# Nightmare-n/GD-MAE

Hardware: AMD Instinct MI355X
Metric: MAE pre-train frames/sec (Waymo-shape, 180k pts, 75% mask) (higher is better)
Workload: dtype bf16

## Files before the change

gd-mae_amd/csrc/dw_grouped.h:

```cpp
#pragma once
#include <hip/hip_runtime.h>

#define GD_DW_MAX_JOBS 9

struct GdDwJob {
  const void* G;
  const void* X;
  int M, N;
  float* part;
  float* colpart;
  int tile0;
  const int* xidx;
  int xidx_stride;
  int x_f32;
  int g_ld, g_cols;
};
struct GdDwGroup {
  GdDwJob job[GD_DW_MAX_JOBS];
  int n_jobs;
  int tiles_total;
  int S;
  long long rows_per_slice;
  long long n_valid;
  int guard_rows = 0;
  int pair_mode = 0;
};

bool gd_dw_group_supported(long long n_pad, int d, int ff);
int gd_dw_group_slices(long long n_pad, int tiles_total);
int gd_dw_group_slices_for(long long n_pad, int tiles_total, int max_wgs);
int gd_dw_pick(long long n, int tiles_total, int max_wgs, long long* n_pad);
int gd_dw_grouped(hipStream_t st, GdDwGroup& A, long long n_pad, long long n_valid);
int gd_dw_grouped_s(hipStream_t st, GdDwGroup& A, long long n_pad, long long n_valid, int S);
```

gd-mae_amd/csrc/dw_grouped.hip:

```cpp
#include "common.h"
#include "dw_grouped.h"
#include <stdlib.h>

typedef float f32x16 __attribute__((ext_vector_type(16)));
typedef __bf16 bf16x8 __attribute__((ext_vector_type(8)));
typedef short s16x4 __attribute__((ext_vector_type(4)));

namespace {
constexpr int kTile = 128;
constexpr int kChunk = 64;
constexpr int kRowBytes = kTile * 2;
constexpr int kStage = kChunk * kRowBytes;

__device__ __forceinline__ int stage_off(int row, int u16) { return row * kRowBytes + (((u16 >> 2) ^ (row & 3)) << 6) + ((u16 & 3) << 4); }

struct Chunk {
  uint4 q0, q1, q2, q3;
};
__device__ __forceinline__ Chunk load_chunk(const unsigned short* __restrict__ p, int ld, unsigned r, unsigned last) {
  Chunk k;
  k.q0 = *reinterpret_cast<const uint4*>(p + (unsigned long long)(r < last ? r : last) * (unsigned)ld);
  k.q1 = *reinterpret_cast<const uint4*>(p + (unsigned long long)(r + 16 < last ? r + 16 : last) * (unsigned)ld);
  k.q2 = *reinterpret_cast<const uint4*>(p + (unsigned long long)(r + 32 < last ? r + 32 : last) * (unsigned)ld);
  k.q3 = *reinterpret_cast<const uint4*>(p + (unsigned long long)(r + 48 < last ? r + 48 : last) * (unsigned)ld);
  return k;
}
__device__ __forceinline__ void zero_chunk_unless(Chunk& k, unsigned keep_mask) {
  k.q0.x &= keep_mask; k.q0.y &= keep_mask; k.q0.z &= keep_mask; k.q0.w &= keep_mask;
  k.q1.x &= keep_mask; k.q1.y &= keep_mask; k.q1.z &= keep_mask; k.q1.w &= keep_mask;
  k.q2.x &= keep_mask; k.q2.y &= keep_mask; k.q2.z &= keep_mask; k.q2.w &= keep_mask;
  k.q3.x &= keep_mask; k.q3.y &= keep_mask; k.q3.z &= keep_mask; k.q3.w &= keep_mask;
}
__device__ __forceinline__ uint4 cvt_f32x8(const float4& a, const float4& b) {
  uint4 q;
  q.x = gd_pack_bf16(a.x, a.y); q.y = gd_pack_bf16(a.z, a.w);
  q.z = gd_pack_bf16(b.x, b.y); q.w = gd_pack_bf16(b.z, b.w);
  return q;
}
struct ChunkIdx {
  int j0, j1, j2, j3;
};
__device__ __forceinline__ ChunkIdx load_chunk_idx(const int* __restrict__ xidx, int stride, unsigned row0, unsigned n_valid, int tid) {
  const unsigned r = row0 + (tid >> 4), lastv = n_valid - 1;
  auto at = [&](unsigned rr) { return xidx[(unsigned long long)(rr < lastv ? rr : lastv) * (unsigned)stride]; };
  ChunkIdx k;
  k.j0 = at(r); k.j1 = at(r + 16); k.j2 = at(r + 32); k.j3 = at(r + 48);
  return k;
}
template <bool F32>
__device__ __forceinline__ Chunk load_chunk_rows(const void* __restrict__ base, int ld, const ChunkIdx& I, int col0, int tid) {
  const int col = col0 + (tid & 15) * 8;
  const long long o0 = (long long)(I.j0 < 0 ? 0 : I.j0) * ld + col, o1 = (long long)(I.j1 < 0 ? 0 : I.j1) * ld + col;
  const long long o2 = (long long)(I.j2 < 0 ? 0 : I.j2) * ld + col, o3 = (long long)(I.j3 < 0 ? 0 : I.j3) * ld + col;
  Chunk k;
  if (F32) {
    const float* f = (const float*)base;
    const float4 a0 = *reinterpret_cast<const float4*>(f + o0), b0 = *reinterpret_cast<const float4*>(f + o0 + 4);
    const float4 a1 = *reinterpret_cast<const float4*>(f + o1), b1 = *reinterpret_cast<const float4*>(f + o1 + 4);
    const float4 a2 = *reinterpret_cast<const float4*>(f + o2), b2 = *reinterpret_cast<const float4*>(f + o2 + 4);
    const float4 a3 = *reinterpret_cast<const float4*>(f + o3), b3 = *reinterpret_cast<const float4*>(f + o3 + 4);
    k.q0 = cvt_f32x8(a0, b0); k.q1 = cvt_f32x8(a1, b1); k.q2 = cvt_f32x8(a2, b2); k.q3 = cvt_f32x8(a3, b3);
  } else {
    const unsigned short* h = (const unsigned short*)base;
    k.q0 = *reinterpret_cast<const uint4*>(h + o0);
    k.q1 = *reinterpret_cast<const uint4*>(h + o1);
    k.q2 = *reinterpret_cast<const uint4*>(h + o2);
    k.q3 = *reinterpret_cast<const uint4*>(h + o3);
  }
  return k;
}
__device__ __forceinline__ unsigned missing_bits(const ChunkIdx& I) {
  return (I.j0 < 0 ? 1u : 0u) | (I.j1 < 0 ? 2u : 0u) | (I.j2 < 0 ? 4u : 0u) | (I.j3 < 0 ? 8u : 0u);
}
__device__ __forceinline__ void zero_missing(Chunk& k, unsigned bits) {
  const unsigned m0 = (bits & 1u) ? 0u : ~0u, m1 = (bits & 2u) ? 0u : ~0u, m2 = (bits & 4u) ? 0u : ~0u, m3 = (bits & 8u) ? 0u : ~0u;
  k.q0.x &= m0; k.q0.y &= m0; k.q0.z &= m0; k.q0.w &= m0;
  k.q1.x &= m1; k.q1.y &= m1; k.q1.z &= m1; k.q1.w &= m1;
  k.q2.x &= m2; k.q2.y &= m2; k.q2.z &= m2; k.q2.w &= m2;
  k.q3.x &= m3; k.q3.y &= m3; k.q3.z &= m3; k.q3.w &= m3;
}
__device__ __forceinline__ void mask_chunk(Chunk& k, long long row0, int tid, long long n_valid) {
  if (row0 + kChunk <= n_valid) return;
  const int r = tid >> 4;
  const uint4 z = make_uint4(0u, 0u, 0u, 0u);
  if (row0 + r >= n_valid) k.q0 = z;
  if (row0 + r + 16 >= n_valid) k.q1 = z;
  if (row0 + r + 32 >= n_valid) k.q2 = z;
  if (row0 + r + 48 >= n_valid) k.q3 = z;
}
__device__ __forceinline__ void store_chunk(unsigned char* __restrict__ lds, int tid, const Chunk& k) {
  const int c = tid & 15, r = tid >> 4;
  unsigned char* p = lds + stage_off(r, c);
  *reinterpret_cast<uint4*>(p) = k.q0;
  *reinterpret_cast<uint4*>(p + 16 * kRowBytes) = k.q1;
  *reinterpret_cast<uint4*>(p + 32 * kRowBytes) = k.q2;
  *reinterpret_cast<uint4*>(p + 48 * kRowBytes) = k.q3;
}
__device__ __forceinline__ void add_bf16x8(const uint4& q, float (&cs)[8]) {
  cs[0] += __uint_as_float(q.x << 16); cs[1] += __uint_as_float(q.x & 0xFFFF0000u);
  cs[2] += __uint_as_float(q.y << 16); cs[3] += __uint_as_float(q.y & 0xFFFF0000u);
  cs[4] += __uint_as_float(q.z << 16); cs[5] += __uint_as_float(q.z & 0xFFFF0000u);
  cs[6] += __uint_as_float(q.w << 16); cs[7] += __uint_as_float(q.w & 0xFFFF0000u);
}
__device__ __forceinline__ bf16x8 frag(const unsigned char* __restrict__ lds, int k0, int col32, int lane) {
  const int i = lane & 15, grp = (lane >> 4) & 1, h = lane >> 5;
  const int row = k0 + 8 * h + (i >> 2);
  const int seg = col32 >> 5;
  const unsigned char* p0 = lds + row * kRowBytes + ((seg ^ (row & 3)) << 6) + 32 * grp + 8 * (i & 3);
  const int row1 = row + 4;
  const unsigned char* p1 = lds + row1 * kRowBytes + ((seg ^ (row1 & 3)) << 6) + 32 * grp + 8 * (i & 3);
  const s16x4 lo = __builtin_amdgcn_ds_read_tr16_b64_v4i16((s16x4 __attribute__((address_space(3)))*)p0);
  const s16x4 hi = __builtin_amdgcn_ds_read_tr16_b64_v4i16((s16x4 __attribute__((address_space(3)))*)p1);
  const uint2 a = __builtin_bit_cast(uint2, lo), b = __builtin_bit_cast(uint2, hi);
  return __builtin_bit_cast(bf16x8, make_uint4(a.x, a.y, b.x, b.y));
}

template <int XM>
__global__ __launch_bounds__(256, 2) void k_dw_grouped(GdDwGroup A) {
  extern __shared__ __attribute__((aligned(16))) unsigned char lds[];
  const int tid = threadIdx.x, lane = tid & 63, wv = tid >> 6;
  const int xcd = blockIdx.x & 7, pos = blockIdx.x >> 3;
  const int sg = pos / A.tiles_total, t = pos - sg * A.tiles_total;
  const int s = sg * 8 + xcd;
  const unsigned short* G = (const unsigned short*)A.job[0].G;
  const unsigned short* X = (const unsigned short*)A.job[0].X;
  float* part = A.job[0].part;
  float* colpart = A.job[0].colpart;
  int M = A.job[0].M, N = A.job[0].N, tile0 = 0;
  const int* xidx = A.job[0].xidx;
  int xstride = A.job[0].xidx_stride, x_f32 = A.job[0].x_f32;
  int g_ld = A.job[0].g_ld, g_cols = A.job[0].g_cols;
#pragma unroll
  for (int j = 1; j < GD_DW_MAX_JOBS; ++j)
    if (j < A.n_jobs && t >= A.job[j].tile0) {
      G = (const unsigned short*)A.job[j].G;
      X = (const unsigned short*)A.job[j].X;
      part = A.job[j].part;
      colpart = A.job[j].colpart;
      M = A.job[j].M;
      N = A.job[j].N;
      tile0 = A.job[j].tile0;
      xidx = A.job[j].xidx;
      xstride = A.job[j].xidx_stride;
      x_f32 = A.job[j].x_f32;
      g_ld = A.job[j].g_ld;
      g_cols = A.job[j].g_cols;
    }
  if (g_ld == 0) g_ld = M;
  if (g_cols == 0) g_cols = M;
  const int tn_count = N / kTile;
  const int tm = (t - tile0) / tn_count, tn = (t - tile0) - tm * tn_count;
  const long long r0 = (long long)s * A.rows_per_slice;
  const int nchunk = (int)(A.rows_per_slice / kChunk);
  const int wm = wv >> 1, wn = wv & 1;
  f32x16 acc[2][2];
#pragma unroll
  for (int i = 0; i < 2; ++i)
#pragma unroll
    for (int j = 0; j < 2; ++j)
#pragma unroll
      for (int e = 0; e < 16; ++e) acc[i][j][e] = 0.f;
  float cs[8];
#pragma unroll
  for (int j = 0; j < 8; ++j) cs[j] = 0.f;
  const bool want_cs = colpart != nullptr && tn == 0;

  const int gcol = tm * kTile, xcol = tn * kTile;
  const unsigned last = A.guard_rows ? (unsigned)(A.n_valid - 1) : 0xFFFFFFFFu;
  const unsigned nv = (unsigned)A.n_valid, rb = (unsigned)r0, rt = (unsigned)r0 + (tid >> 4);
  const int c8 = (tid & 15) * 8;
  const bool gkeep = gcol + c8 < g_cols;
  const unsigned short* gp = G + (gkeep ? gcol + c8 : 0);
  const unsigned gmask = gkeep ? 0xFFFFFFFFu : 0u;
  const unsigned short* xp = X + xcol + c8;
  ChunkIdx i0 = {-1, -1, -1, -1}, i1 = {-1, -1, -1, -1};
  unsigned miss0 = 0u, miss1 = 0u;
  auto load_x = [&](unsigned chunk, ChunkIdx& I, unsigned& miss) {
    if constexpr (XM == 0) {
      return load_chunk(xp, N, rt + chunk * kChunk, last);
    } else {
      const Chunk k = load_chunk_rows<XM == 2>(X, N, I, xcol, tid);
      miss = missing_bits(I);
      I = load_chunk_idx(xidx, xstride, rb + (chunk + 2) * kChunk, nv, tid);
      return k;
    }
  };
  auto load_g = [&](unsigned chunk) { return load_chunk(gp, g_ld, rt + chunk * kChunk, last); };
  if constexpr (XM != 0) {
    i0 = load_chunk_idx(xidx, xstride, rb, nv, tid);
    i1 = load_chunk_idx(xidx, xstride, rb + kChunk, nv, tid);
  }
  auto compute = [&](const unsigned char* bg, const unsigned char* bx) {
#pragma unroll
    for (int ks = 0; ks < kChunk / 16; ++ks) {
      const bf16x8 a0 = frag(bg, 16 * ks, wm * 64, lane), a1 = frag(bg, 16 * ks, wm * 64 + 32, lane);
      const bf16x8 b0 = frag(bx, 16 * ks, wn * 64, lane), b1 = frag(bx, 16 * ks, wn * 64 + 32, lane);
      acc[0][0] = __builtin_amdgcn_mfma_f32_32x32x16_bf16(a0, b0, acc[0][0], 0, 0, 0);
      acc[0][1] = __builtin_amdgcn_mfma_f32_32x32x16_bf16(a0, b1, acc[0][1], 0, 0, 0);
      acc[1][0] = __builtin_amdgcn_mfma_f32_32x32x16_bf16(a1, b0, acc[1][0], 0, 0, 0);
      acc[1][1] = __builtin_amdgcn_mfma_f32_32x32x16_bf16(a1, b1, acc[1][1], 0, 0, 0);
    }
  };
  unsigned char* bufg0 = lds;
  unsigned char* bufx0 = lds + kStage;
  unsigned char* bufg1 = lds + 2 * kStage;
  unsigned char* bufx1 = lds + 3 * kStage;
  const long long r_end = r0 + A.rows_per_slice < A.n_valid ? r0 + A.rows_per_slice : A.n_valid;
  Chunk g0 = load_g(0), x0 = load_x(0, i0, miss0);
  __builtin_amdgcn_sched_barrier(0);
  const unsigned c1 = nchunk > 1 ? 1u : 0u;
  Chunk g1 = load_g(c1), x1 = load_x(c1, i1, miss1);
  __builtin_amdgcn_sched_barrier(0);
  for (int c = 0; c < nchunk; c += 2) {
    mask_chunk(g0, r0 + (long long)c * kChunk, tid, r_end);
    mask_chunk(x0, r0 + (long long)c * kChunk, tid, r_end);
    zero_chunk_unless(g0, gmask);
    if constexpr (XM != 0) zero_missing(x0, miss0);
    store_chunk(bufg0, tid, g0);
    store_chunk(bufx0, tid, x0);
    if (want_cs) {
      add_bf16x8(g0.q0, cs); add_bf16x8(g0.q1, cs); add_bf16x8(g0.q2, cs); add_bf16x8(g0.q3, cs);
    }
    __syncthreads();
    {
      const unsigned cn = c + 2 < nchunk ? c + 2 : nchunk - 1;
      g0 = load_g(cn);
      x0 = load_x(cn, i0, miss0);
    }
    __builtin_amdgcn_sched_barrier(0);
    compute(bufg0, bufx0);
    mask_chunk(g1, r0 + (long long)(c + 1) * kChunk, tid, r_end);
    mask_chunk(x1, r0 + (long long)(c + 1) * kChunk, tid, r_end);
    zero_chunk_unless(g1, gmask);
    if constexpr (XM != 0) zero_missing(x1, miss1);
    store_chunk(bufg1, tid, g1);
    store_chunk(bufx1, tid, x1);
    if (want_cs) {
      add_bf16x8(g1.q0, cs); add_bf16x8(g1.q1, cs); add_bf16x8(g1.q2, cs); add_bf16x8(g1.q3, cs);
    }
    __syncthreads();
    {
      const unsigned cn = c + 3 < nchunk ? c + 3 : nchunk - 1;
      g1 = load_g(cn);
      x1 = load_x(cn, i1, miss1);
    }
    __builtin_amdgcn_sched_barrier(0);
    compute(bufg1, bufx1);
  }
  float* out = part + ((long long)s * M + tm * kTile + wm * 64) * N + tn * kTile + wn * 64;
#pragma unroll
  for (int i = 0; i < 2; ++i)
#pragma unroll
    for (int j = 0; j < 2; ++j)
#pragma unroll
      for (int e = 0; e < 16; ++e) {
        const int m = i * 32 + (e & 3) + 8 * (e >> 2) + 4 * (lane >> 5);
        out[(long long)m * N + j * 32 + (lane & 31)] = acc[i][j][e];
      }
  if (want_cs) {
    __syncthreads();
    float* red = reinterpret_cast<float*>(lds);
    const int c = tid & 15, r = tid >> 4;
#pragma unroll
    for (int j = 0; j < 8; ++j) red[r * kTile + c * 8 + j] = cs[j];
    __syncthreads();
    if (tid < kTile) {
      float tsum = 0.f;
#pragma unroll
      for (int rr = 0; rr < 16; ++rr) tsum += red[rr * kTile + tid];
      colpart[(long long)s * M + tm * kTile + tid] = tsum;
    }
  }
}

struct Chunk2 {
  uint4 q0, q1;
};
__device__ __forceinline__ Chunk2 load_chunk2(const unsigned short* __restrict__ p, int ld, unsigned r, unsigned last) {
  Chunk2 k;
  k.q0 = *reinterpret_cast<const uint4*>(p + (unsigned long long)(r < last ? r : last) * (unsigned)ld);
  k.q1 = *reinterpret_cast<const uint4*>(p + (unsigned long long)(r + 32 < last ? r + 32 : last) * (unsigned)ld);
  return k;
}
struct ChunkIdx2 {
  int j0, j1;
};
__device__ __forceinline__ ChunkIdx2 load_chunk_idx2(const int* __restrict__ xidx, int stride, unsigned row0, unsigned n_valid, int tid) {
  const unsigned r = row0 + (tid >> 4), lastv = n_valid - 1;
  ChunkIdx2 k;
  k.j0 = xidx[(unsigned long long)(r < lastv ? r : lastv) * (unsigned)stride];
  k.j1 = xidx[(unsigned long long)(r + 32 < lastv ? r + 32 : lastv) * (unsigned)stride];
  return k;
}
template <bool F32>
__device__ __forceinline__ Chunk2 load_chunk_rows2(const void* __restrict__ base, int ld, const ChunkIdx2& I, int col0, int tid) {
  const int col = col0 + (tid & 15) * 8;
  const long long o0 = (long long)(I.j0 < 0 ? 0 : I.j0) * ld + col, o1 = (long long)(I.j1 < 0 ? 0 : I.j1) * ld + col;
  Chunk2 k;
  if (F32) {
    const float* f = (const float*)base;
    const float4 a0 = *reinterpret_cast<const float4*>(f + o0), b0 = *reinterpret_cast<const float4*>(f + o0 + 4);
    const float4 a1 = *reinterpret_cast<const float4*>(f + o1), b1 = *reinterpret_cast<const float4*>(f + o1 + 4);
    k.q0 = cvt_f32x8(a0, b0); k.q1 = cvt_f32x8(a1, b1);
  } else {
    const unsigned short* h = (const unsigned short*)base;
    k.q0 = *reinterpret_cast<const uint4*>(h + o0);
    k.q1 = *reinterpret_cast<const uint4*>(h + o1);
  }
  return k;
}
__device__ __forceinline__ void and_u4(uint4& q, unsigned m) { q.x &= m; q.y &= m; q.z &= m; q.w &= m; }
__device__ __forceinline__ void clear_chunk2(Chunk2& k, long long row0, int tid, long long n_valid, unsigned miss_bits) {
  const int r = tid >> 4;
  and_u4(k.q0, (row0 + r < n_valid && !(miss_bits & 1u)) ? ~0u : 0u);
  and_u4(k.q1, (row0 + r + 32 < n_valid && !(miss_bits & 2u)) ? ~0u : 0u);
}
__device__ __forceinline__ void store_chunk2(unsigned char* __restrict__ lds, int tid, const Chunk2& k) {
  const int c = tid & 15, r = tid >> 4;
  unsigned char* p = lds + stage_off(r, c);
  *reinterpret_cast<uint4*>(p) = k.q0;
  *reinterpret_cast<uint4*>(p + 32 * kRowBytes) = k.q1;
}

template <int XM>
__global__ __launch_bounds__(512, 1) void k_dw_grouped2(GdDwGroup A) {
  extern __shared__ __attribute__((aligned(16))) unsigned char lds[];
  const int tid = threadIdx.x, lane = tid & 63, wv = tid >> 6;
  const int xcd = blockIdx.x & 7, pos = blockIdx.x >> 3;
  const int sg = pos / A.tiles_total, t = pos - sg * A.tiles_total;
  const int s = sg * 8 + xcd;
  const bool taps = A.pair_mode == 2;
  const unsigned short* G = (const unsigned short*)A.job[0].G;
  const void* X = A.job[0].X;
  float* part = A.job[0].part;
  float* colpart = A.job[0].colpart;
  int M = A.job[0].M, N = A.job[0].N, tile0 = 0;
  const int* xidx = A.job[0].xidx;
  int xstride = A.job[0].xidx_stride;
  const int* xidx_b = A.n_jobs > 1 ? A.job[1].xidx : nullptr;
  float* part_b = A.n_jobs > 1 ? A.job[1].part : nullptr;
#pragma unroll
  for (int j = 1; j < GD_DW_MAX_JOBS; ++j)
    if (j < A.n_jobs && t >= A.job[j].tile0) {
      G = (const unsigned short*)A.job[j].G;
      X = A.job[j].X;
      part = A.job[j].part;
      colpart = A.job[j].colpart;
      M = A.job[j].M;
      N = A.job[j].N;
      tile0 = A.job[j].tile0;
      xidx = A.job[j].xidx;
      xstride = A.job[j].xidx_stride;
      xidx_b = j + 1 < A.n_jobs ? A.job[j + 1 < GD_DW_MAX_JOBS ? j + 1 : j].xidx : nullptr;
      part_b = j + 1 < A.n_jobs ? A.job[j + 1 < GD_DW_MAX_JOBS ? j + 1 : j].part : nullptr;
    }
  const int tn_count = taps ? N / kTile : N / (2 * kTile);
  const int tm = (t - tile0) / tn_count, tq = (t - tile0) - tm * tn_count;
  const int xcol_a = taps ? tq * kTile : tq * 2 * kTile, xcol_b = taps ? xcol_a : xcol_a + kTile;
  if (!taps) { xidx_b = xidx; part_b = part; }
  const bool have_b = part_b != nullptr;
  if (!have_b) xidx_b = xidx;
  const long long r0 = (long long)s * A.rows_per_slice;
  const int nchunk = (int)(A.rows_per_slice / kChunk);
  const int sub = wv >> 2, wm = (wv >> 1) & 1, wn = wv & 1;
  f32x16 acc[2][2];
#pragma unroll
  for (int i = 0; i < 2; ++i)
#pragma unroll
    for (int j = 0; j < 2; ++j)
#pragma unroll
      for (int e = 0; e < 16; ++e) acc[i][j][e] = 0.f;
  float cs[8];
#pragma unroll
  for (int j = 0; j < 8; ++j) cs[j] = 0.f;
  const bool want_cs = colpart != nullptr && tq == 0;
  const int gcol = tm * kTile;
  const unsigned last = A.guard_rows ? (unsigned)(A.n_valid - 1) : 0xFFFFFFFFu;
  const unsigned nv = (unsigned)A.n_valid, rb = (unsigned)r0, rt = (unsigned)r0 + (tid >> 4);
  const int c8 = (tid & 15) * 8;
  const unsigned short* gp = G + gcol + c8;
  const unsigned short* xpa = (const unsigned short*)X + xcol_a + c8;
  const unsigned short* xpb = (const unsigned short*)X + xcol_b + c8;
  ChunkIdx2 ia0 = {-1, -1}, ia1 = {-1, -1}, ib0 = {-1, -1}, ib1 = {-1, -1};
  unsigned ma0 = 0u, ma1 = 0u, mb0 = 0u, mb1 = 0u;
  auto load_xa = [&](unsigned chunk, ChunkIdx2& I, unsigned& miss) {
    if constexpr (XM == 0) {
      return load_chunk2(xpa, N, rt + chunk * kChunk, last);
    } else {
      const Chunk2 k = load_chunk_rows2<XM == 2>(X, N, I, xcol_a, tid);
      miss = (I.j0 < 0 ? 1u : 0u) | (I.j1 < 0 ? 2u : 0u);
      I = load_chunk_idx2(xidx, xstride, rb + (chunk + 2) * kChunk, nv, tid);
      return k;
    }
  };
  auto load_xb = [&](unsigned chunk, ChunkIdx2& I, unsigned& miss) {
    if constexpr (XM == 0) {
      return load_chunk2(xpb, N, rt + chunk * kChunk, last);
    } else {
      const Chunk2 k = load_chunk_rows2<XM == 2>(X, N, I, xcol_b, tid);
      miss = (I.j0 < 0 ? 1u : 0u) | (I.j1 < 0 ? 2u : 0u);
      I = load_chunk_idx2(xidx_b, xstride, rb + (chunk + 2) * kChunk, nv, tid);
      return k;
    }
  };
  auto load_g = [&](unsigned chunk) { return load_chunk2(gp, M, rt + chunk * kChunk, last); };
  if constexpr (XM != 0) {
    ia0 = load_chunk_idx2(xidx, xstride, rb, nv, tid);
    ib0 = load_chunk_idx2(xidx_b, xstride, rb, nv, tid);
    ia1 = load_chunk_idx2(xidx, xstride, rb + kChunk, nv, tid);
    ib1 = load_chunk_idx2(xidx_b, xstride, rb + kChunk, nv, tid);
  }
  auto compute = [&](const unsigned char* bg, const unsigned char* bx) {
#pragma unroll
    for (int ks = 0; ks < kChunk / 16; ++ks) {
      const bf16x8 a0 = frag(bg, 16 * ks, wm * 64, lane), a1 = frag(bg, 16 * ks, wm * 64 + 32, lane);
      const bf16x8 b0 = frag(bx, 16 * ks, wn * 64, lane), b1 = frag(bx, 16 * ks, wn * 64 + 32, lane);
      acc[0][0] = __builtin_amdgcn_mfma_f32_32x32x16_bf16(a0, b0, acc[0][0], 0, 0, 0);
      acc[0][1] = __builtin_amdgcn_mfma_f32_32x32x16_bf16(a0, b1, acc[0][1], 0, 0, 0);
      acc[1][0] = __builtin_amdgcn_mfma_f32_32x32x16_bf16(a1, b0, acc[1][0], 0, 0, 0);
      acc[1][1] = __builtin_amdgcn_mfma_f32_32x32x16_bf16(a1, b1, acc[1][1], 0, 0, 0);
    }
  };
  unsigned char* const buf0 = lds;
  unsigned char* const buf1 = lds + 3 * kStage;
  const long long r_end = r0 + A.rows_per_slice < A.n_valid ? r0 + A.rows_per_slice : A.n_valid;
  Chunk2 g0 = load_g(0), xa0 = load_xa(0, ia0, ma0), xb0 = load_xb(0, ib0, mb0);
  __builtin_amdgcn_sched_barrier(0);
  const unsigned c1 = nchunk > 1 ? 1u : 0u;
  Chunk2 g1 = load_g(c1), xa1 = load_xa(c1, ia1, ma1), xb1 = load_xb(c1, ib1, mb1);
  __builtin_amdgcn_sched_barrier(0);
  for (int c = 0; c < nchunk; c += 2) {
    {
      const long long cr = r0 + (long long)c * kChunk;
      clear_chunk2(g0, cr, tid, r_end, 0u);
      clear_chunk2(xa0, cr, tid, r_end, XM != 0 ? ma0 : 0u);
      clear_chunk2(xb0, cr, tid, r_end, XM != 0 ? mb0 : 0u);
    }
    store_chunk2(buf0, tid, g0);
    store_chunk2(buf0 + kStage, tid, xa0);
    store_chunk2(buf0 + 2 * kStage, tid, xb0);
    if (want_cs) { add_bf16x8(g0.q0, cs); add_bf16x8(g0.q1, cs); }
    __syncthreads();
    {
      const unsigned cn = c + 2 < nchunk ? c + 2 : nchunk - 1;
      g0 = load_g(cn);
      xa0 = load_xa(cn, ia0, ma0);
      xb0 = load_xb(cn, ib0, mb0);
    }
    __builtin_amdgcn_sched_barrier(0);
    compute(buf0, buf0 + (1 + sub) * kStage);
    {
      const long long cr = r0 + (long long)(c + 1) * kChunk;
      clear_chunk2(g1, cr, tid, r_end, 0u);
      clear_chunk2(xa1, cr, tid, r_end, XM != 0 ? ma1 : 0u);
      clear_chunk2(xb1, cr, tid, r_end, XM != 0 ? mb1 : 0u);
    }
    store_chunk2(buf1, tid, g1);
    store_chunk2(buf1 + kStage, tid, xa1);
    store_chunk2(buf1 + 2 * kStage, tid, xb1);
    if (want_cs) { add_bf16x8(g1.q0, cs); add_bf16x8(g1.q1, cs); }
    __syncthreads();
    {
      const unsigned cn = c + 3 < nchunk ? c + 3 : nchunk - 1;
      g1 = load_g(cn);
      xa1 = load_xa(cn, ia1, ma1);
      xb1 = load_xb(cn, ib1, mb1);
    }
    __builtin_amdgcn_sched_barrier(0);
    compute(buf1, buf1 + (1 + sub) * kStage);
  }
  if (sub == 0 || have_b) {
    float* out = (sub ? part_b : part) + ((long long)s * M + tm * kTile + wm * 64) * N + (sub ? xcol_b : xcol_a) + wn * 64;
#pragma unroll
    for (int i = 0; i < 2; ++i)
#pragma unroll
      for (int j = 0; j < 2; ++j)
#pragma unroll
        for (int e = 0; e < 16; ++e) {
          const int m = i * 32 + (e & 3) + 8 * (e >> 2) + 4 * (lane >> 5);
          out[(long long)m * N + j * 32 + (lane & 31)] = acc[i][j][e];
        }
  }
  if (want_cs) {
    __syncthreads();
    float* red = reinterpret_cast<float*>(lds);
    const int c = tid & 15, r = tid >> 4;
#pragma unroll
    for (int j = 0; j < 8; ++j) red[r * kTile + c * 8 + j] = cs[j];
    __syncthreads();
    if (tid < kTile) {
      float tsum = 0.f;
#pragma unroll
      for (int rr = 0; rr < 32; ++rr) tsum += red[rr * kTile + tid];
      colpart[(long long)s * M + tm * kTile + tid] = tsum;
    }
  }
}
}

bool gd_dw_group_supported(long long n_pad, int d, int ff) {
  return d % kTile == 0 && ff % kTile == 0 && d <= 512 && ff <= 1024 && n_pad > 0 && n_pad % (8 * kChunk) == 0;
}
int gd_dw_group_slices(long long n_pad, int tiles_total) {
  static const int pinned = getenv("GDMAE_DW_WGS") ? atoi(getenv("GDMAE_DW_WGS")) : 0;
  static const long long short_rows = getenv("GDMAE_DW_ROWS") ? atoll(getenv("GDMAE_DW_ROWS")) : 32768;
  const int wgs = pinned > 0 ? pinned : (n_pad < short_rows ? 256 : 512);
  return gd_dw_group_slices_for(n_pad, tiles_total, wgs);
}
int gd_dw_pick(long long n, int tiles_total, int max_wgs, long long* n_pad) {
  int S = 8;
  while (S < 64 && (long long)tiles_total * S * 2 <= max_wgs && n / (S * 2) >= 4 * kChunk) S *= 2;
  const long long g = (long long)S * kChunk;
  *n_pad = (n + g - 1) / g * g;
  if (*n_pad < g) *n_pad = g;
  return S;
}
int gd_dw_group_slices_for(long long n_pad, int tiles_total, int max_wgs) {
  int S = 8;
  while (S < 64 && (long long)tiles_total * S * 2 <= max_wgs && n_pad % ((long long)S * 2 * kChunk) == 0 && n_pad / (S * 2) >= 2 * kChunk) S *= 2;
  return S;
}

int gd_dw_grouped(hipStream_t st, GdDwGroup& A, long long n_pad, long long n_valid) { return gd_dw_grouped_s(st, A, n_pad, n_valid, 0); }
int gd_dw_grouped_s(hipStream_t st, GdDwGroup& A, long long n_pad, long long n_valid, int S) {
  GD_REQUIRE(A.n_jobs >= 1 && A.n_jobs <= GD_DW_MAX_JOBS, "dw_grouped: job count");
  int tiles = 0;
  for (int j = 0; j < A.n_jobs; ++j) {
    GD_REQUIRE(A.job[j].M % kTile == 0 && A.job[j].N % kTile == 0, "dw_grouped: M, N must be multiples of 128");
    A.job[j].tile0 = tiles;
    tiles += (A.job[j].M / kTile) * (A.job[j].N / kTile);
  }
  A.tiles_total = tiles;
  GD_REQUIRE(n_pad % (8 * kChunk) == 0, "dw_grouped: rows must be a multiple of 512");
  A.S = S > 0 ? S : gd_dw_group_slices(n_pad, tiles);
  GD_REQUIRE(A.S % 8 == 0 && n_pad % ((long long)A.S * kChunk) == 0, "dw_grouped: slices must be a multiple of 8 that divides the row chunks");
  A.rows_per_slice = n_pad / A.S;
  A.n_valid = n_valid;
  double by = 0.0, fl = 0.0, l2 = 0.0;
  for (int j = 0; j < A.n_jobs; ++j) {
    bool g_new = true, x_new = true;
    for (int i = 0; i < j; ++i) {
      g_new = g_new && A.job[i].G != A.job[j].G;
      x_new = x_new && A.job[i].X != A.job[j].X;
    }
    const double gcols = A.job[j].g_cols ? A.job[j].g_cols : A.job[j].M, xb = A.job[j].x_f32 ? 4.0 : 2.0;
    const double part = 4.0 * A.S * (double)A.job[j].M * A.job[j].N;
    by += (g_new ? 2.0 * n_valid * gcols : 0.0) + (x_new ? xb * n_valid * A.job[j].N : 0.0) + (A.job[j].xidx ? 4.0 * n_valid : 0.0) + part;
    l2 += 2.0 * n_valid * gcols + xb * n_valid * A.job[j].N + (A.job[j].xidx ? 4.0 * n_valid : 0.0) + part;
    fl += 2.0 * n_valid * (double)A.job[j].M * A.job[j].N;
  }
  GdTimed timed(GD_T_DW_GROUPED, st, by, fl, l2);
  GD_REQUIRE(n_valid >= 0 && n_pad < (1ll << 31), "dw_grouped: row count");
  if (n_valid == 0) {
    for (int j = 0; j < A.n_jobs; ++j) {
      GD_CHECK(hipMemsetAsync(A.job[j].part, 0, (size_t)A.S * A.job[j].M * A.job[j].N * sizeof(float), st));
      if (A.job[j].colpart) GD_CHECK(hipMemsetAsync(A.job[j].colpart, 0, (size_t)A.S * A.job[j].M * sizeof(float), st));
    }
    return 0;
  }
  const int xm = A.job[0].xidx ? (A.job[0].x_f32 ? 2 : 1) : 0;
  for (int j = 1; j < A.n_jobs; ++j)
    GD_REQUIRE((A.job[j].xidx ? (A.job[j].x_f32 ? 2 : 1) : 0) == xm, "dw_grouped: the jobs of a launch share the X addressing mode");
  static const bool pair_ok = getenv("GDMAE_DW_PAIR") && atoi(getenv("GDMAE_DW_PAIR")) != 0;
  int mode = 0;
  if (pair_ok) {
    bool plain = true, cols = true, same = true;
    for (int j = 0; j < A.n_jobs; ++j) {
      const GdDwJob& q = A.job[j];
      plain = plain && q.g_ld == 0 && q.g_cols == 0;
      cols = cols && q.N % (2 * kTile) == 0;
      same = same && q.G == A.job[0].G && q.X == A.job[0].X && q.M == A.job[0].M && q.N == A.job[0].N && q.xidx != nullptr &&
             q.xidx_stride == A.job[0].xidx_stride && q.colpart == nullptr;
    }
    if (plain && cols) mode = 1;
    else if (plain && same && A.n_jobs >= 2) mode = 2;
  }
  if (mode != 0) {
    A.pair_mode = mode;
    int pt = 0;
    for (int j = 0; j < A.n_jobs; ++j) {
      if (mode == 1) {
        A.job[j].tile0 = pt;
        pt += (A.job[j].M / kTile) * (A.job[j].N / (2 * kTile));
      } else if ((j & 1) == 0) {
        A.job[j].tile0 = pt;
        pt += (A.job[j].M / kTile) * (A.job[j].N / kTile);
      } else {
        A.job[j].tile0 = 0x7FFFFFFF;
      }
    }
    A.tiles_total = pt;
    static bool once[3] = {false, false, false};
    if (!once[xm]) {
      const void* fn = xm == 0 ? (const void*)k_dw_grouped2<0> : (xm == 1 ? (const void*)k_dw_grouped2<1> : (const void*)k_dw_grouped2<2>);
      GD_CHECK(hipFuncSetAttribute(fn, hipFuncAttributeMaxDynamicSharedMemorySize, 6 * kStage));
      once[xm] = true;
    }
    const dim3 grid2((unsigned)(pt * A.S));
    if (xm == 0) hipLaunchKernelGGL(k_dw_grouped2<0>, grid2, dim3(512), 6 * kStage, st, A);
    else if (xm == 1) hipLaunchKernelGGL(k_dw_grouped2<1>, grid2, dim3(512), 6 * kStage, st, A);
    else hipLaunchKernelGGL(k_dw_grouped2<2>, grid2, dim3(512), 6 * kStage, st, A);
    GD_LAUNCH_CHECK();
    return 0;
  }
  const dim3 grid((unsigned)(tiles * A.S));
  if (xm == 0) hipLaunchKernelGGL(k_dw_grouped<0>, grid, dim3(256), 4 * kStage, st, A);
  else if (xm == 1) hipLaunchKernelGGL(k_dw_grouped<1>, grid, dim3(256), 4 * kStage, st, A);
  else hipLaunchKernelGGL(k_dw_grouped<2>, grid, dim3(256), 4 * kStage, st, A);
  GD_LAUNCH_CHECK();
  return 0;
}

namespace {
__global__ __launch_bounds__(256) void k_dw_reduce(const float* __restrict__ part, int S, long long P, float* __restrict__ dst) {
  for (long long i = blockIdx.x * (long long)blockDim.x + threadIdx.x; i < P; i += (long long)gridDim.x * blockDim.x) {
    float a = 0.f;
    for (int s = 0; s < S; ++s) a += part[(long long)s * P + i];
    dst[i] = a;
  }
}
}
extern "C" size_t gdmae_dw_gemm_workspace_bytes(long long rows, int M, int N) {
  const int S = gd_dw_group_slices(rows, (M / kTile) * (N / kTile));
  return gd_align((size_t)S * M * N * sizeof(float)) + gd_align((size_t)S * M * sizeof(float));
}
extern "C" int gdmae_dw_gemm(const void* G, const void* X, long long rows, int M, int N, float* dW, float* dbias, void* workspace,
                             void* stream) {
  hipStream_t st = (hipStream_t)stream;
  GD_REQUIRE(M % kTile == 0 && N % kTile == 0 && rows > 0 && rows % (8 * kChunk) == 0, "dw_gemm: M, N multiples of 128, rows a multiple of 512");
  GdDwGroup A;
  A.n_jobs = 1;
  const int S = gd_dw_group_slices(rows, (M / kTile) * (N / kTile));
  float* part = (float*)workspace;
  float* colpart = (float*)((char*)workspace + gd_align((size_t)S * M * N * sizeof(float)));
  A.job[0] = GdDwJob{G, X, M, N, part, dbias ? colpart : nullptr, 0};
  {
    const int rc = gd_dw_grouped(st, A, rows, rows);
    if (rc != 0) return rc;
  }
  hipLaunchKernelGGL(k_dw_reduce, dim3(256), dim3(256), 0, st, (const float*)part, A.S, (long long)M * N, dW);
  GD_LAUNCH_CHECK();
  if (dbias) {
    hipLaunchKernelGGL(k_dw_reduce, dim3(4), dim3(256), 0, st, (const float*)colpart, A.S, (long long)M, dbias);
    GD_LAUNCH_CHECK();
  }
  return 0;
}
```

Before: 1065.

## Replace pair-mode weight-gradient kernel with default-on wide 128x256 tile kernel

Removes the opt-in 512-thread pair kernel and adds a 256-thread kernel where each workgroup computes two 128x128 output tiles that share one operand. The pairs can be adjacent columns, adjacent rows (G reused as the second operand), or two tap jobs sharing G. Staging uses 32-row sub-chunks in three slots with double buffering. The wide path is chosen by default when the tile-by-slice count exceeds the device's resident workgroup capacity. The aim is to halve operand reloads and raise MFMA work per LDS byte, at the cost of more accumulator registers and possibly lower occupancy.

New measurement: 1067 (median of 6 runs). No clear change (+0.2%).

```diff
diff --git a/gd-mae_amd/csrc/dw_grouped.h b/gd-mae_amd/csrc/dw_grouped.h
--- a/gd-mae_amd/csrc/dw_grouped.h
+++ b/gd-mae_amd/csrc/dw_grouped.h
@@ -2,6 +2,12 @@
 #include <hip/hip_runtime.h>
 
 #define GD_DW_MAX_JOBS 9
+
+#define GD_DW_COLS 0
+#define GD_DW_ROWS 1
+#define GD_DW_TAPS 2
+#define GD_DW_SINGLE 3
+#define GD_DW_PARTNER 4
 
 struct GdDwJob {
   const void* G;
@@ -14,6 +20,7 @@
   int xidx_stride;
   int x_f32;
   int g_ld, g_cols;
+  int form = GD_DW_COLS;
 };
 struct GdDwGroup {
   GdDwJob job[GD_DW_MAX_JOBS];
@@ -23,7 +30,6 @@
   long long rows_per_slice;
   long long n_valid;
   int guard_rows = 0;
-  int pair_mode = 0;
 };
 
 bool gd_dw_group_supported(long long n_pad, int d, int ff);
diff --git a/gd-mae_amd/csrc/dw_grouped.hip b/gd-mae_amd/csrc/dw_grouped.hip
--- a/gd-mae_amd/csrc/dw_grouped.hip
+++ b/gd-mae_amd/csrc/dw_grouped.hip
@@ -9,11 +9,86 @@
 namespace {
 constexpr int kTile = 128;
 constexpr int kChunk = 64;
+constexpr int kSub = 32;
 constexpr int kRowBytes = kTile * 2;
-constexpr int kStage = kChunk * kRowBytes;
+constexpr int kSlot = kSub * kRowBytes;
+constexpr int kStage = 3 * kSlot;
+constexpr int kLds = 2 * kStage;
 
 __device__ __forceinline__ int stage_off(int row, int u16) { return row * kRowBytes + (((u16 >> 2) ^ (row & 3)) << 6) + ((u16 & 3) << 4); }
 
+struct Piece {
+  uint4 q0, q1;
+};
+struct Stage {
+  Piece s0, s1, s2;
+};
+__device__ __forceinline__ Piece load_piece(const unsigned short* __restrict__ p, unsigned ld, unsigned r, unsigned last) {
+  Piece k;
+  k.q0 = *reinterpret_cast<const uint4*>(p + (unsigned long long)(r < last ? r : last) * ld);
+  k.q1 = *reinterpret_cast<const uint4*>(p + (unsigned long long)(r + 16 < last ? r + 16 : last) * ld);
+  return k;
+}
+__device__ __forceinline__ void and_u4(uint4& q, unsigned m) { q.x &= m; q.y &= m; q.z &= m; q.w &= m; }
+__device__ __forceinline__ uint4 cvt_f32x8(const float4& a, const float4& b) {
+  uint4 q;
+  q.x = gd_pack_bf16(a.x, a.y); q.y = gd_pack_bf16(a.z, a.w);
+  q.z = gd_pack_bf16(b.x, b.y); q.w = gd_pack_bf16(b.z, b.w);
+  return q;
+}
+struct PieceIdx {
+  int j0, j1;
+};
+__device__ __forceinline__ PieceIdx load_piece_idx(const int* __restrict__ xidx, unsigned stride, unsigned r, unsigned lastv) {
+  PieceIdx k;
+  k.j0 = xidx[(unsigned long long)(r < lastv ? r : lastv) * stride];
+  k.j1 = xidx[(unsigned long long)(r + 16 < lastv ? r + 16 : lastv) * stride];
+  return k;
+}
+__device__ __forceinline__ Piece load_piece_rows(const unsigned short* __restrict__ base, int ld, const PieceIdx& I, int col) {
+  const long long o0 = (long long)(I.j0 < 0 ? 0 : I.j0) * ld + col, o1 = (long long)(I.j1 < 0 ? 0 : I.j1) * ld + col;
+  Piece k;
+  k.q0 = *reinterpret_cast<const uint4*>(base + o0);
+  k.q1 = *reinterpret_cast<const uint4*>(base + o1);
+  return k;
+}
+__device__ __forceinline__ unsigned missing_bits(const PieceIdx& I) { return (I.j0 < 0 ? 1u : 0u) | (I.j1 < 0 ? 2u : 0u); }
+__device__ __forceinline__ void zero_missing(Piece& k, unsigned bits) {
+  and_u4(k.q0, (bits & 1u) ? 0u : ~0u);
+  and_u4(k.q1, (bits & 2u) ? 0u : ~0u);
+}
+__device__ __forceinline__ void mask_stage(Stage& k, long long row0, int tid, long long n_valid) {
+  if (row0 + kSub <= n_valid) return;
+  const int r = tid >> 4;
+  const unsigned m0 = row0 + r < n_valid ? ~0u : 0u, m1 = row0 + r + 16 < n_valid ? ~0u : 0u;
+  and_u4(k.s0.q0, m0); and_u4(k.s1.q0, m0); and_u4(k.s2.q0, m0);
+  and_u4(k.s0.q1, m1); and_u4(k.s1.q1, m1); and_u4(k.s2.q1, m1);
+}
+__device__ __forceinline__ void store_piece(unsigned char* __restrict__ p, const Piece& k) {
+  *reinterpret_cast<uint4*>(p) = k.q0;
+  *reinterpret_cast<uint4*>(p + 16 * kRowBytes) = k.q1;
+}
+__device__ __forceinline__ void add_bf16x8(const uint4& q, float (&cs)[8]) {
+  cs[0] += __uint_as_float(q.x << 16); cs[1] += __uint_as_float(q.x & 0xFFFF0000u);
+  cs[2] += __uint_as_float(q.y << 16); cs[3] += __uint_as_float(q.y & 0xFFFF0000u);
+  cs[4] += __uint_as_float(q.z << 16); cs[5] += __uint_as_float(q.z & 0xFFFF0000u);
+  cs[6] += __uint_as_float(q.w << 16); cs[7] += __uint_as_float(q.w & 0xFFFF0000u);
+}
+__device__ __forceinline__ void add_piece(const Piece& k, float (&cs)[8]) { add_bf16x8(k.q0, cs); add_bf16x8(k.q1, cs); }
+__device__ __forceinline__ bf16x8 frag(const unsigned char* __restrict__ lds, int k0, int col32, int lane) {
+  const int i = lane & 15, grp = (lane >> 4) & 1, h = lane >> 5;
+  const int row = k0 + 8 * h + (i >> 2);
+  const int seg = col32 >> 5;
+  const unsigned char* p0 = lds + row * kRowBytes + ((seg ^ (row & 3)) << 6) + 32 * grp + 8 * (i & 3);
+  const int row1 = row + 4;
+  const unsigned char* p1 = lds + row1 * kRowBytes + ((seg ^ (row1 & 3)) << 6) + 32 * grp + 8 * (i & 3);
+  const s16x4 lo = __builtin_amdgcn_ds_read_tr16_b64_v4i16((s16x4 __attribute__((address_space(3)))*)p0);
+  const s16x4 hi = __builtin_amdgcn_ds_read_tr16_b64_v4i16((s16x4 __attribute__((address_space(3)))*)p1);
+  const uint2 a = __builtin_bit_cast(uint2, lo), b = __builtin_bit_cast(uint2, hi);
+  return __builtin_bit_cast(bf16x8, make_uint4(a.x, a.y, b.x, b.y));
+}
+
+constexpr int kChunkBytes = kChunk * kRowBytes;
 struct Chunk {
   uint4 q0, q1, q2, q3;
 };
@@ -30,12 +105,6 @@
   k.q1.x &= keep_mask; k.q1.y &= keep_mask; k.q1.z &= keep_mask; k.q1.w &= keep_mask;
   k.q2.x &= keep_mask; k.q2.y &= keep_mask; k.q2.z &= keep_mask; k.q2.w &= keep_mask;
   k.q3.x &= keep_mask; k.q3.y &= keep_mask; k.q3.z &= keep_mask; k.q3.w &= keep_mask;
-}
-__device__ __forceinline__ uint4 cvt_f32x8(const float4& a, const float4& b) {
-  uint4 q;
-  q.x = gd_pack_bf16(a.x, a.y); q.y = gd_pack_bf16(a.z, a.w);
-  q.z = gd_pack_bf16(b.x, b.y); q.w = gd_pack_bf16(b.z, b.w);
-  return q;
 }
 struct ChunkIdx {
   int j0, j1, j2, j3;
@@ -96,27 +165,9 @@
   *reinterpret_cast<uint4*>(p + 32 * kRowBytes) = k.q2;
   *reinterpret_cast<uint4*>(p + 48 * kRowBytes) = k.q3;
 }
-__device__ __forceinline__ void add_bf16x8(const uint4& q, float (&cs)[8]) {
-  cs[0] += __uint_as_float(q.x << 16); cs[1] += __uint_as_float(q.x & 0xFFFF0000u);
-  cs[2] += __uint_as_float(q.y << 16); cs[3] += __uint_as_float(q.y & 0xFFFF0000u);
-  cs[4] += __uint_as_float(q.z << 16); cs[5] += __uint_as_float(q.z & 0xFFFF0000u);
-  cs[6] += __uint_as_float(q.w << 16); cs[7] += __uint_as_float(q.w & 0xFFFF0000u);
-}
-__device__ __forceinline__ bf16x8 frag(const unsigned char* __restrict__ lds, int k0, int col32, int lane) {
-  const int i = lane & 15, grp = (lane >> 4) & 1, h = lane >> 5;
-  const int row = k0 + 8 * h + (i >> 2);
-  const int seg = col32 >> 5;
-  const unsigned char* p0 = lds + row * kRowBytes + ((seg ^ (row & 3)) << 6) + 32 * grp + 8 * (i & 3);
-  const int row1 = row + 4;
-  const unsigned char* p1 = lds + row1 * kRowBytes + ((seg ^ (row1 & 3)) << 6) + 32 * grp + 8 * (i & 3);
-  const s16x4 lo = __builtin_amdgcn_ds_read_tr16_b64_v4i16((s16x4 __attribute__((address_space(3)))*)p0);
-  const s16x4 hi = __builtin_amdgcn_ds_read_tr16_b64_v4i16((s16x4 __attribute__((address_space(3)))*)p1);
-  const uint2 a = __builtin_bit_cast(uint2, lo), b = __builtin_bit_cast(uint2, hi);
-  return __builtin_bit_cast(bf16x8, make_uint4(a.x, a.y, b.x, b.y));
-}
 
 template <int XM>
-__global__ __launch_bounds__(256, 2) void k_dw_grouped(GdDwGroup A) {
+__global__ __launch_bounds__(256, 2) void k_dw_tile(GdDwGroup A) {
   extern __shared__ __attribute__((aligned(16))) unsigned char lds[];
   const int tid = threadIdx.x, lane = tid & 63, wv = tid >> 6;
   const int xcd = blockIdx.x & 7, pos = blockIdx.x >> 3;
@@ -202,9 +253,9 @@
     }
   };
   unsigned char* bufg0 = lds;
-  unsigned char* bufx0 = lds + kStage;
-  unsigned char* bufg1 = lds + 2 * kStage;
-  unsigned char* bufx1 = lds + 3 * kStage;
+  unsigned char* bufx0 = lds + kChunkBytes;
+  unsigned char* bufg1 = lds + 2 * kChunkBytes;
+  unsigned char* bufx1 = lds + 3 * kChunkBytes;
   const long long r_end = r0 + A.rows_per_slice < A.n_valid ? r0 + A.rows_per_slice : A.n_valid;
   Chunk g0 = load_g(0), x0 = load_x(0, i0, miss0);
   __builtin_amdgcn_sched_barrier(0);
@@ -273,228 +324,214 @@
   }
 }
 
-struct Chunk2 {
-  uint4 q0, q1;
-};
-__device__ __forceinline__ Chunk2 load_chunk2(const unsigned short* __restrict__ p, int ld, unsigned r, unsigned last) {
-  Chunk2 k;
-  k.q0 = *reinterpret_cast<const uint4*>(p + (unsigned long long)(r < last ? r : last) * (unsigned)ld);
-  k.q1 = *reinterpret_cast<const uint4*>(p + (unsigned long long)(r + 32 < last ? r + 32 : last) * (unsigned)ld);
-  return k;
-}
-struct ChunkIdx2 {
-  int j0, j1;
-};
-__device__ __forceinline__ ChunkIdx2 load_chunk_idx2(const int* __restrict__ xidx, int stride, unsigned row0, unsigned n_valid, int tid) {
-  const unsigned r = row0 + (tid >> 4), lastv = n_valid - 1;
-  ChunkIdx2 k;
-  k.j0 = xidx[(unsigned long long)(r < lastv ? r : lastv) * (unsigned)stride];
-  k.j1 = xidx[(unsigned long long)(r + 32 < lastv ? r + 32 : lastv) * (unsigned)stride];
-  return k;
-}
-template <bool F32>
-__device__ __forceinline__ Chunk2 load_chunk_rows2(const void* __restrict__ base, int ld, const ChunkIdx2& I, int col0, int tid) {
-  const int col = col0 + (tid & 15) * 8;
-  const long long o0 = (long long)(I.j0 < 0 ? 0 : I.j0) * ld + col, o1 = (long long)(I.j1 < 0 ? 0 : I.j1) * ld + col;
-  Chunk2 k;
-  if (F32) {
-    const float* f = (const float*)base;
-    const float4 a0 = *reinterpret_cast<const float4*>(f + o0), b0 = *reinterpret_cast<const float4*>(f + o0 + 4);
-    const float4 a1 = *reinterpret_cast<const float4*>(f + o1), b1 = *reinterpret_cast<const float4*>(f + o1 + 4);
-    k.q0 = cvt_f32x8(a0, b0); k.q1 = cvt_f32x8(a1, b1);
-  } else {
-    const unsigned short* h = (const unsigned short*)base;
-    k.q0 = *reinterpret_cast<const uint4*>(h + o0);
-    k.q1 = *reinterpret_cast<const uint4*>(h + o1);
-  }
-  return k;
-}
-__device__ __forceinline__ void and_u4(uint4& q, unsigned m) { q.x &= m; q.y &= m; q.z &= m; q.w &= m; }
-__device__ __forceinline__ void clear_chunk2(Chunk2& k, long long row0, int tid, long long n_valid, unsigned miss_bits) {
-  const int r = tid >> 4;
-  and_u4(k.q0, (row0 + r < n_valid && !(miss_bits & 1u)) ? ~0u : 0u);
-  and_u4(k.q1, (row0 + r + 32 < n_valid && !(miss_bits & 2u)) ? ~0u : 0u);
-}
-__device__ __forceinline__ void store_chunk2(unsigned char* __restrict__ lds, int tid, const Chunk2& k) {
-  const int c = tid & 15, r = tid >> 4;
-  unsigned char* p = lds + stage_off(r, c);
-  *reinterpret_cast<uint4*>(p) = k.q0;
-  *reinterpret_cast<uint4*>(p + 32 * kRowBytes) = k.q1;
-}
-
 template <int XM>
-__global__ __launch_bounds__(512, 1) void k_dw_grouped2(GdDwGroup A) {
+__global__ __launch_bounds__(256, 2) void k_dw_grouped(GdDwGroup A) {
+  static_assert(XM == 0 || XM == 1, "wide tiles: plain or bf16-gathered X");
   extern __shared__ __attribute__((aligned(16))) unsigned char lds[];
   const int tid = threadIdx.x, lane = tid & 63, wv = tid >> 6;
   const int xcd = blockIdx.x & 7, pos = blockIdx.x >> 3;
   const int sg = pos / A.tiles_total, t = pos - sg * A.tiles_total;
   const int s = sg * 8 + xcd;
-  const bool taps = A.pair_mode == 2;
   const unsigned short* G = (const unsigned short*)A.job[0].G;
-  const void* X = A.job[0].X;
+  const unsigned short* X = (const unsigned short*)A.job[0].X;
   float* part = A.job[0].part;
   float* colpart = A.job[0].colpart;
-  int M = A.job[0].M, N = A.job[0].N, tile0 = 0;
+  int M = A.job[0].M, N = A.job[0].N, tile0 = 0, form = A.job[0].form;
   const int* xidx = A.job[0].xidx;
   int xstride = A.job[0].xidx_stride;
-  const int* xidx_b = A.n_jobs > 1 ? A.job[1].xidx : nullptr;
-  float* part_b = A.n_jobs > 1 ? A.job[1].part : nullptr;
+  int g_ld = A.job[0].g_ld, g_cols = A.job[0].g_cols;
+  const int* xidx_b = A.job[1].xidx;
+  float* part_b = A.job[1].part;
 #pragma unroll
   for (int j = 1; j < GD_DW_MAX_JOBS; ++j)
     if (j < A.n_jobs && t >= A.job[j].tile0) {
       G = (const unsigned short*)A.job[j].G;
-      X = A.job[j].X;
+      X = (const unsigned short*)A.job[j].X;
       part = A.job[j].part;
       colpart = A.job[j].colpart;
       M = A.job[j].M;
       N = A.job[j].N;
       tile0 = A.job[j].tile0;
+      form = A.job[j].form;
       xidx = A.job[j].xidx;
       xstride = A.job[j].xidx_stride;
-      xidx_b = j + 1 < A.n_jobs ? A.job[j + 1 < GD_DW_MAX_JOBS ? j + 1 : j].xidx : nullptr;
-      part_b = j + 1 < A.n_jobs ? A.job[j + 1 < GD_DW_MAX_JOBS ? j + 1 : j].part : nullptr;
-    }
-  const int tn_count = taps ? N / kTile : N / (2 * kTile);
-  const int tm = (t - tile0) / tn_count, tq = (t - tile0) - tm * tn_count;
-  const int xcol_a = taps ? tq * kTile : tq * 2 * kTile, xcol_b = taps ? xcol_a : xcol_a + kTile;
-  if (!taps) { xidx_b = xidx; part_b = part; }
-  const bool have_b = part_b != nullptr;
-  if (!have_b) xidx_b = xidx;
+      g_ld = A.job[j].g_ld;
+      g_cols = A.job[j].g_cols;
+      xidx_b = A.job[j + 1 < GD_DW_MAX_JOBS ? j + 1 : j].xidx;
+      part_b = A.job[j + 1 < GD_DW_MAX_JOBS ? j + 1 : j].part;
+    }
+  if (g_ld == 0) g_ld = M;
+  if (g_cols == 0) g_cols = M;
+  const int mt = M / kTile, nt = N / kTile, u = t - tile0;
+  int tm_a, tn_a, tm_b, tn_b;
+  bool have_b;
+  if (form == GD_DW_COLS) {
+    const int nw = (nt + 1) >> 1;
+    tm_a = u / nw; tn_a = 2 * (u - tm_a * nw); tm_b = tm_a; tn_b = tn_a + 1; have_b = tn_b < nt;
+  } else if (form == GD_DW_ROWS) {
+    const int q = u / nt;
+    tn_a = u - q * nt; tm_a = 2 * q; tm_b = tm_a + 1; tn_b = tn_a; have_b = tm_b < mt;
+  } else {
+    tm_a = u / nt; tn_a = u - tm_a * nt; tm_b = tm_a; tn_b = tn_a; have_b = form == GD_DW_TAPS;
+  }
+  if (form != GD_DW_TAPS) { xidx_b = xidx; part_b = part; }
+  const bool shared_x = XM == 0 && form == GD_DW_ROWS;
+  if (!have_b) { tm_b = tm_a; tn_b = tn_a; xidx_b = xidx; }
   const long long r0 = (long long)s * A.rows_per_slice;
-  const int nchunk = (int)(A.rows_per_slice / kChunk);
-  const int sub = wv >> 2, wm = (wv >> 1) & 1, wn = wv & 1;
-  f32x16 acc[2][2];
+  const int nsub = (int)(A.rows_per_slice / kSub);
+
+  f32x16 acc[2][4];
 #pragma unroll
   for (int i = 0; i < 2; ++i)
 #pragma unroll
-    for (int j = 0; j < 2; ++j)
+    for (int j = 0; j < 4; ++j)
 #pragma unroll
       for (int e = 0; e < 16; ++e) acc[i][j][e] = 0.f;
-  float cs[8];
-#pragma unroll
-  for (int j = 0; j < 8; ++j) cs[j] = 0.f;
-  const bool want_cs = colpart != nullptr && tq == 0;
-  const int gcol = tm * kTile;
+  float csa[8], csb[8];
+#pragma unroll
+  for (int j = 0; j < 8; ++j) { csa[j] = 0.f; csb[j] = 0.f; }
+  const bool want_a = XM == 0 && colpart != nullptr && tn_a == 0, want_b = want_a && shared_x && have_b;
+
   const unsigned last = A.guard_rows ? (unsigned)(A.n_valid - 1) : 0xFFFFFFFFu;
-  const unsigned nv = (unsigned)A.n_valid, rb = (unsigned)r0, rt = (unsigned)r0 + (tid >> 4);
+  const unsigned lastv = (unsigned)A.n_valid - 1u, rt = (unsigned)r0 + (tid >> 4);
   const int c8 = (tid & 15) * 8;
-  const unsigned short* gp = G + gcol + c8;
-  const unsigned short* xpa = (const unsigned short*)X + xcol_a + c8;
-  const unsigned short* xpb = (const unsigned short*)X + xcol_b + c8;
-  ChunkIdx2 ia0 = {-1, -1}, ia1 = {-1, -1}, ib0 = {-1, -1}, ib1 = {-1, -1};
-  unsigned ma0 = 0u, ma1 = 0u, mb0 = 0u, mb1 = 0u;
-  auto load_xa = [&](unsigned chunk, ChunkIdx2& I, unsigned& miss) {
+  const unsigned keep_a = tm_a * kTile + c8 < g_cols ? ~0u : 0u, keep_b = tm_b * kTile + c8 < g_cols ? ~0u : 0u;
+  const bool narrow = XM == 0 && g_cols < M;
+  const unsigned short* gpa = G + (keep_a ? tm_a * kTile + c8 : 0);
+  const unsigned short* gpb = G + (keep_b ? tm_b * kTile + c8 : 0);
+  const int xcol_a = tn_a * kTile + c8, xcol_b = tn_b * kTile + c8;
+  const unsigned short* p1 = X + xcol_a;
+  const unsigned short* p2 = shared_x ? gpb : X + xcol_b;
+  const unsigned ld2 = shared_x ? (unsigned)g_ld : (unsigned)N;
+  PieceIdx ia0 = {-1, -1}, ia1 = {-1, -1}, ib0 = {-1, -1}, ib1 = {-1, -1};
+  unsigned m0 = 0u, m1 = 0u;
+  auto load = [&](unsigned c, PieceIdx& Ia, PieceIdx& Ib, unsigned& miss) {
+    Stage k;
+    const unsigned r = rt + c * kSub;
+    k.s0 = load_piece(gpa, (unsigned)g_ld, r, last);
     if constexpr (XM == 0) {
-      return load_chunk2(xpa, N, rt + chunk * kChunk, last);
+      k.s1 = load_piece(p1, (unsigned)N, r, last);
+      k.s2 = load_piece(p2, ld2, r, last);
     } else {
-      const Chunk2 k = load_chunk_rows2<XM == 2>(X, N, I, xcol_a, tid);
-      miss = (I.j0 < 0 ? 1u : 0u) | (I.j1 < 0 ? 2u : 0u);
-      I = load_chunk_idx2(xidx, xstride, rb + (chunk + 2) * kChunk, nv, tid);
-      return k;
-    }
+      const unsigned rn = r + 2 * kSub;
+      k.s1 = load_piece_rows(X, N, Ia, xcol_a);
+      k.s2 = load_piece_rows(X, N, Ib, xcol_b);
+      miss = missing_bits(Ia) | missing_bits(Ib) << 2;
+      Ib = load_piece_idx(xidx_b, (unsigned)xstride, rn, lastv);
+      Ia = load_piece_idx(xidx, (unsigned)xstride, rn, lastv);
+    }
+    return k;
   };
-  auto load_xb = [&](unsigned chunk, ChunkIdx2& I, unsigned& miss) {
-    if constexpr (XM == 0) {
-      return load_chunk2(xpb, N, rt + chunk * kChunk, last);
-    } else {
-      const Chunk2 k = load_chunk_rows2<XM == 2>(X, N, I, xcol_b, tid);
-      miss = (I.j0 < 0 ? 1u : 0u) | (I.j1 < 0 ? 2u : 0u);
-      I = load_chunk_idx2(xidx_b, xstride, rb + (chunk + 2) * kChunk, nv, tid);
-      return k;
+  if constexpr (XM != 0) {
+    ia0 = load_piece_idx(xidx, (unsigned)xstride, rt, lastv);
+    ia1 = load_piece_idx(xidx, (unsigned)xstride, rt + kSub, lastv);
+    ib0 = load_piece_idx(xidx_b, (unsigned)xstride, rt, lastv);
+    ib1 = load_piece_idx(xidx_b, (unsigned)xstride, rt + kSub, lastv);
+  }
+  const int sub = wv >> 1, half = wv & 1;
+  const bool active = have_b || sub == 0;
+  const int a_off = sub && shared_x ? 2 * kSlot : 0, b_off = sub && !shared_x ? 2 * kSlot : kSlot;
+  auto compute = [&](const unsigned char* buf) {
+    if (!active) return;
+    const unsigned char* ba = buf + a_off;
+    const unsigned char* bb = buf + b_off;
+#pragma unroll
+    for (int ks = 0; ks < kSub / 16; ++ks) {
+      const bf16x8 a0 = frag(ba, 16 * ks, half * 64, lane), a1 = frag(ba, 16 * ks, half * 64 + 32, lane);
+#pragma unroll
+      for (int j = 0; j < 4; ++j) {
+        const bf16x8 b = frag(bb, 16 * ks, 32 * j, lane);
+        acc[0][j] = __builtin_amdgcn_mfma_f32_32x32x16_bf16(a0, b, acc[0][j], 0, 0, 0);
+        acc[1][j] = __builtin_amdgcn_mfma_f32_32x32x16_bf16(a1, b, acc[1][j], 0, 0, 0);
+      }
     }
   };
-  auto load_g = [&](unsigned chunk) { return load_chunk2(gp, M, rt + chunk * kChunk, last); };
-  if constexpr (XM != 0) {
-    ia0 = load_chunk_idx2(xidx, xstride, rb, nv, tid);
-    ib0 = load_chunk_idx2(xidx_b, xstride, rb, nv, tid);
-    ia1 = load_chunk_idx2(xidx, xstride, rb + kChunk, nv, tid);
-    ib1 = load_chunk_idx2(xidx_b, xstride, rb + kChunk, nv, tid);
-  }
-  auto compute = [&](const unsigned char* bg, const unsigned char* bx) {
-#pragma unroll
-    for (int ks = 0; ks < kChunk / 16; ++ks) {
-      const bf16x8 a0 = frag(bg, 16 * ks, wm * 64, lane), a1 = frag(bg, 16 * ks, wm * 64 + 32, lane);
-      const bf16x8 b0 = frag(bx, 16 * ks, wn * 64, lane), b1 = frag(bx, 16 * ks, wn * 64 + 32, lane);
-      acc[0][0] = __builtin_amdgcn_mfma_f32_32x32x16_bf16(a0, b0, acc[0][0], 0, 0, 0);
-      acc[0][1] = __builtin_amdgcn_mfma_f32_32x32x16_bf16(a0, b1, acc[0][1], 0, 0, 0);
-      acc[1][0] = __builtin_amdgcn_mfma_f32_32x32x16_bf16(a1, b0, acc[1][0], 0, 0, 0);
-      acc[1][1] = __builtin_amdgcn_mfma_f32_32x32x16_bf16(a1, b1, acc[1][1], 0, 0, 0);
-    }
+  const int st_off = stage_off(tid >> 4, tid & 15);
+  const long long r_end = r0 + A.rows_per_slice < A.n_valid ? r0 + A.rows_per_slice : A.n_valid;
+  auto stage = [&](unsigned char* buf, Stage& k, int c, unsigned miss) {
+    mask_stage(k, r0 + (long long)c * kSub, tid, r_end);
+    if (narrow) {
+      and_u4(k.s0.q0, keep_a); and_u4(k.s0.q1, keep_a);
+      if (shared_x) { and_u4(k.s2.q0, keep_b); and_u4(k.s2.q1, keep_b); }
+    }
+    if constexpr (XM != 0) {
+      zero_missing(k.s1, miss);
+      zero_missing(k.s2, miss >> 2);
+    }
+    store_piece(buf + st_off, k.s0);
+    store_piece(buf + kSlot + st_off, k.s1);
+    store_piece(buf + 2 * kSlot + st_off, k.s2);
+    if (want_a) add_piece(k.s0, csa);
+    if (want_b) add_piece(k.s2, csb);
   };
   unsigned char* const buf0 = lds;
-  unsigned char* const buf1 = lds + 3 * kStage;
-  const long long r_end = r0 + A.rows_per_slice < A.n_valid ? r0 + A.rows_per_slice : A.n_valid;
-  Chunk2 g0 = load_g(0), xa0 = load_xa(0, ia0, ma0), xb0 = load_xb(0, ib0, mb0);
+  unsigned char* const buf1 = lds + kStage;
+  Stage st0 = load(0, ia0, ib0, m0);
   __builtin_amdgcn_sched_barrier(0);
-  const unsigned c1 = nchunk > 1 ? 1u : 0u;
-  Chunk2 g1 = load_g(c1), xa1 = load_xa(c1, ia1, ma1), xb1 = load_xb(c1, ib1, mb1);
+  Stage st1 = load(1, ia1, ib1, m1);
   __builtin_amdgcn_sched_barrier(0);
-  for (int c = 0; c < nchunk; c += 2) {
-    {
-      const long long cr = r0 + (long long)c * kChunk;
-      clear_chunk2(g0, cr, tid, r_end, 0u);
-      clear_chunk2(xa0, cr, tid, r_end, XM != 0 ? ma0 : 0u);
-      clear_chunk2(xb0, cr, tid, r_end, XM != 0 ? mb0 : 0u);
-    }
-    store_chunk2(buf0, tid, g0);
-    store_chunk2(buf0 + kStage, tid, xa0);
-    store_chunk2(buf0 + 2 * kStage, tid, xb0);
-    if (want_cs) { add_bf16x8(g0.q0, cs); add_bf16x8(g0.q1, cs); }
+  auto phase = [&](unsigned char* buf, Stage& k, int c, PieceIdx& Ia, PieceIdx& Ib, unsigned& miss) {
+    stage(buf, k, c, miss);
     __syncthreads();
-    {
-      const unsigned cn = c + 2 < nchunk ? c + 2 : nchunk - 1;
-      g0 = load_g(cn);
-      xa0 = load_xa(cn, ia0, ma0);
-      xb0 = load_xb(cn, ib0, mb0);
-    }
+    k = load(c + 2 < nsub ? c + 2 : nsub - 1, Ia, Ib, miss);
     __builtin_amdgcn_sched_barrier(0);
-    compute(buf0, buf0 + (1 + sub) * kStage);
-    {
-      const long long cr = r0 + (long long)(c + 1) * kChunk;
-      clear_chunk2(g1, cr, tid, r_end, 0u);
-      clear_chunk2(xa1, cr, tid, r_end, XM != 0 ? ma1 : 0u);
-      clear_chunk2(xb1, cr, tid, r_end, XM != 0 ? mb1 : 0u);
-    }
-    store_chunk2(buf1, tid, g1);
-    store_chunk2(buf1 + kStage, tid, xa1);
-    store_chunk2(buf1 + 2 * kStage, tid, xb1);
-    if (want_cs) { add_bf16x8(g1.q0, cs); add_bf16x8(g1.q1, cs); }
-    __syncthreads();
-    {
-      const unsigned cn = c + 3 < nchunk ? c + 3 : nchunk - 1;
-      g1 = load_g(cn);
-      xa1 = load_xa(cn, ia1, ma1);
-      xb1 = load_xb(cn, ib1, mb1);
-    }
-    __builtin_amdgcn_sched_barrier(0);
-    compute(buf1, buf1 + (1 + sub) * kStage);
-  }
-  if (sub == 0 || have_b) {
-    float* out = (sub ? part_b : part) + ((long long)s * M + tm * kTile + wm * 64) * N + (sub ? xcol_b : xcol_a) + wn * 64;
+    compute(buf);
+  };
+  for (int c = 0; c < nsub; c += 4) {
+    phase(buf0, st0, c, ia0, ib0, m0);
+    phase(buf1, st1, c + 1, ia1, ib1, m1);
+    phase(buf0, st0, c + 2, ia0, ib0, m0);
+    phase(buf1, st1, c + 3, ia1, ib1, m1);
+  }
+  if (active) {
+    float* out = (sub ? part_b : part) + ((long long)s * M + (sub ? tm_b : tm_a) * kTile + half * 64) * N + (sub ? tn_b : tn_a) * kTile;
 #pragma unroll
     for (int i = 0; i < 2; ++i)
 #pragma unroll
-      for (int j = 0; j < 2; ++j)
+      for (int j = 0; j < 4; ++j)
 #pragma unroll
         for (int e = 0; e < 16; ++e) {
           const int m = i * 32 + (e & 3) + 8 * (e >> 2) + 4 * (lane >> 5);
           out[(long long)m * N + j * 32 + (lane & 31)] = acc[i][j][e];
         }
   }
-  if (want_cs) {
+  if (want_a) {
     __syncthreads();
     float* red = reinterpret_cast<float*>(lds);
     const int c = tid & 15, r = tid >> 4;
 #pragma unroll
-    for (int j = 0; j < 8; ++j) red[r * kTile + c * 8 + j] = cs[j];
+    for (int j = 0; j < 8; ++j) red[r * kTile + c * 8 + j] = csa[j];
+    if (want_b) {
+#pragma unroll
+      for (int j = 0; j < 8; ++j) red[16 * kTile + r * kTile + c * 8 + j] = csb[j];
+    }
     __syncthreads();
     if (tid < kTile) {
       float tsum = 0.f;
 #pragma unroll
-      for (int rr = 0; rr < 32; ++rr) tsum += red[rr * kTile + tid];
-      colpart[(long long)s * M + tm * kTile + tid] = tsum;
-    }
-  }
+      for (int rr = 0; rr < 16; ++rr) tsum += red[rr * kTile + tid];
+      colpart[(long long)s * M + tm_a * kTile + tid] = tsum;
+    } else if (want_b) {
+      const int col = tid - kTile;
+      float tsum = 0.f;
+#pragma unroll
+      for (int rr = 0; rr < 16; ++rr) tsum += red[16 * kTile + rr * kTile + col];
+      colpart[(long long)s * M + tm_b * kTile + col] = tsum;
+    }
+  }
+}
+
+int dw_slots() {
+  static const int slots = [] {
+    int dev = 0, cus = 0, occ = 0;
+    if (hipGetDevice(&dev) != hipSuccess || hipDeviceGetAttribute(&cus, hipDeviceAttributeMultiprocessorCount, dev) != hipSuccess ||
+        hipOccupancyMaxActiveBlocksPerMultiprocessor(&occ, k_dw_grouped<0>, 256, kLds) != hipSuccess || cus * occ <= 0) {
+      (void)hipGetLastError();
+      return 512;
+    }
+    return cus * occ;
+  }();
+  return slots;
 }
 }
 
@@ -524,16 +561,50 @@
 int gd_dw_grouped(hipStream_t st, GdDwGroup& A, long long n_pad, long long n_valid) { return gd_dw_grouped_s(st, A, n_pad, n_valid, 0); }
 int gd_dw_grouped_s(hipStream_t st, GdDwGroup& A, long long n_pad, long long n_valid, int S) {
   GD_REQUIRE(A.n_jobs >= 1 && A.n_jobs <= GD_DW_MAX_JOBS, "dw_grouped: job count");
+  const int xm = A.job[0].xidx ? (A.job[0].x_f32 ? 2 : 1) : 0;
+  for (int j = 1; j < A.n_jobs; ++j)
+    GD_REQUIRE((A.job[j].xidx ? (A.job[j].x_f32 ? 2 : 1) : 0) == xm, "dw_grouped: the jobs of a launch share the X addressing mode");
+  for (int j = 0; j < A.n_jobs; ++j)
+    GD_REQUIRE(xm == 0 || (!A.job[j].colpart && (A.job[j].g_cols == 0 || A.job[j].g_cols == A.job[j].M)),
+               "dw_grouped: gathered jobs take no column sums and read G at full width");
+  int tiles128 = 0;
+  for (int j = 0; j < A.n_jobs; ++j) {
+    GD_REQUIRE(A.job[j].M % kTile == 0 && A.job[j].N % kTile == 0, "dw_grouped: M, N must be multiples of 128");
+    tiles128 += (A.job[j].M / kTile) * (A.job[j].N / kTile);
+  }
+  GD_REQUIRE(n_pad % (8 * kChunk) == 0, "dw_grouped: rows must be a multiple of 512");
+  A.S = S > 0 ? S : gd_dw_group_slices(n_pad, tiles128);
+  GD_REQUIRE(A.S % 8 == 0 && n_pad % ((long long)A.S * kChunk) == 0, "dw_grouped: slices must be a multiple of 8 that divides the row chunks");
+  static const int wide_mode = getenv("GDMAE_DW_WIDE") ? atoi(getenv("GDMAE_DW_WIDE")) : 1;
+  const bool wide = xm != 2 && (wide_mode == 2 || (wide_mode == 1 && (long long)tiles128 * A.S > dw_slots()));
   int tiles = 0;
   for (int j = 0; j < A.n_jobs; ++j) {
-    GD_REQUIRE(A.job[j].M % kTile == 0 && A.job[j].N % kTile == 0, "dw_grouped: M, N must be multiples of 128");
-    A.job[j].tile0 = tiles;
-    tiles += (A.job[j].M / kTile) * (A.job[j].N / kTile);
+    GdDwJob& q = A.job[j];
+    const int mt = q.M / kTile, nt = q.N / kTile;
+    q.tile0 = tiles;
+    if (!wide) {
+      q.form = GD_DW_SINGLE;
+      tiles += mt * nt;
+    } else if (nt >= 2) {
+      q.form = GD_DW_COLS;
+      tiles += mt * ((nt + 1) / 2);
+    } else if (j + 1 < A.n_jobs && q.xidx && A.job[j + 1].G == q.G && A.job[j + 1].X == q.X && A.job[j + 1].M == q.M && A.job[j + 1].N == q.N &&
+               A.job[j + 1].xidx && A.job[j + 1].xidx_stride == q.xidx_stride && !q.colpart && !A.job[j + 1].colpart && A.job[j + 1].g_ld == q.g_ld &&
+               A.job[j + 1].g_cols == q.g_cols) {
+      q.form = GD_DW_TAPS;
+      tiles += mt * nt;
+      ++j;
+      A.job[j].form = GD_DW_PARTNER;
+      A.job[j].tile0 = 0x7FFFFFFF;
+    } else if (xm == 0 && mt >= 2) {
+      q.form = GD_DW_ROWS;
+      tiles += (mt + 1) / 2 * nt;
+    } else {
+      q.form = GD_DW_SINGLE;
+      tiles += mt * nt;
+    }
   }
   A.tiles_total = tiles;
-  GD_REQUIRE(n_pad % (8 * kChunk) == 0, "dw_grouped: rows must be a multiple of 512");
-  A.S = S > 0 ? S : gd_dw_group_slices(n_pad, tiles);
-  GD_REQUIRE(A.S % 8 == 0 && n_pad % ((long long)A.S * kChunk) == 0, "dw_grouped: slices must be a multiple of 8 that divides the row chunks");
   A.rows_per_slice = n_pad / A.S;
   A.n_valid = n_valid;
   double by = 0.0, fl = 0.0, l2 = 0.0;
@@ -558,55 +629,13 @@
     }
     return 0;
   }
-  const int xm = A.job[0].xidx ? (A.job[0].x_f32 ? 2 : 1) : 0;
-  for (int j = 1; j < A.n_jobs; ++j)
-    GD_REQUIRE((A.job[j].xidx ? (A.job[j].x_f32 ? 2 : 1) : 0) == xm, "dw_grouped: the jobs of a launch share the X addressing mode");
-  static const bool pair_ok = getenv("GDMAE_DW_PAIR") && atoi(getenv("GDMAE_DW_PAIR")) != 0;
-  int mode = 0;
-  if (pair_ok) {
-    bool plain = true, cols = true, same = true;
-    for (int j = 0; j < A.n_jobs; ++j) {
-      const GdDwJob& q = A.job[j];
-      plain = plain && q.g_ld == 0 && q.g_cols == 0;
-      cols = cols && q.N % (2 * kTile) == 0;
-      same = same && q.G == A.job[0].G && q.X == A.job[0].X && q.M == A.job[0].M && q.N == A.job[0].N && q.xidx != nullptr &&
-             q.xidx_stride == A.job[0].xidx_stride && q.colpart == nullptr;
-    }
-    if (plain && cols) mode = 1;
-    else if (plain && same && A.n_jobs >= 2) mode = 2;
-  }
-  if (mode != 0) {
-    A.pair_mode = mode;
-    int pt = 0;
-    for (int j = 0; j < A.n_jobs; ++j) {
-      if (mode == 1) {
-        A.job[j].tile0 = pt;
-        pt += (A.job[j].M / kTile) * (A.job[j].N / (2 * kTile));
-      } else if ((j & 1) == 0) {
-        A.job[j].tile0 = pt;
-        pt += (A.job[j].M / kTile) * (A.job[j].N / kTile);
-      } else {
-        A.job[j].tile0 = 0x7FFFFFFF;
-      }
-    }
-    A.tiles_total = pt;
-    static bool once[3] = {false, false, false};
-    if (!once[xm]) {
-      const void* fn = xm == 0 ? (const void*)k_dw_grouped2<0> : (xm == 1 ? (const void*)k_dw_grouped2<1> : (const void*)k_dw_grouped2<2>);
-      GD_CHECK(hipFuncSetAttribute(fn, hipFuncAttributeMaxDynamicSharedMemorySize, 6 * kStage));
-      once[xm] = true;
-    }
-    const dim3 grid2((unsigned)(pt * A.S));
-    if (xm == 0) hipLaunchKernelGGL(k_dw_grouped2<0>, grid2, dim3(512), 6 * kStage, st, A);
-    else if (xm == 1) hipLaunchKernelGGL(k_dw_grouped2<1>, grid2, dim3(512), 6 * kStage, st, A);
-    else hipLaunchKernelGGL(k_dw_grouped2<2>, grid2, dim3(512), 6 * kStage, st, A);
-    GD_LAUNCH_CHECK();
-    return 0;
-  }
   const dim3 grid((unsigned)(tiles * A.S));
-  if (xm == 0) hipLaunchKernelGGL(k_dw_grouped<0>, grid, dim3(256), 4 * kStage, st, A);
-  else if (xm == 1) hipLaunchKernelGGL(k_dw_grouped<1>, grid, dim3(256), 4 * kStage, st, A);
-  else hipLaunchKernelGGL(k_dw_grouped<2>, grid, dim3(256), 4 * kStage, st, A);
+  if (!wide) {
+    if (xm == 0) hipLaunchKernelGGL(k_dw_tile<0>, grid, dim3(256), 4 * kChunkBytes, st, A);
+    else if (xm == 1) hipLaunchKernelGGL(k_dw_tile<1>, grid, dim3(256), 4 * kChunkBytes, st, A);
+    else hipLaunchKernelGGL(k_dw_tile<2>, grid, dim3(256), 4 * kChunkBytes, st, A);
+  } else if (xm == 0) hipLaunchKernelGGL(k_dw_grouped<0>, grid, dim3(256), kLds, st, A);
+  else hipLaunchKernelGGL(k_dw_grouped<1>, grid, dim3(256), kLds, st, A);
   GD_LAUNCH_CHECK();
   return 0;
 }
```
